# ZheyuanXie/CUDA-Path-Tracer-Denoising

Measured on AMD Instinct MI355X. Metric: SVGF Mpixels/s (full pipeline) at 1080p; à-trous HBM GB/s vs roofline, higher is better.
Workload: dtype f32; 1 GPU; cornell-like 1920x1080, full SVGF (temporal + 5 a-trous levels, history_level 1), static camera, steady-state history; one independent sequence per GPU; width=1920, height=1080, atrous_levels=5, parallelism=replicas1

## Files before the change

### cuda-path-tracer-denoising_amd/csrc/svgf_kernels.h

```cpp
#pragma once
#include <hip/hip_runtime.h>
#include <hip/hip_ext.h>
#include <mutex>

#ifdef SVGF_BUILD_EXPERIMENTS
int svgf_exp_get(const char *name, int dflt);
#define SVGF_TUNE(name, dflt) svgf_exp_get(name, dflt)
#else
#define SVGF_TUNE(name, dflt) (dflt)
#endif

struct SvgfLaunchEvents { hipEvent_t start, stop; };
extern thread_local SvgfLaunchEvents g_svgf_launch_events;
#define SVGF_LAUNCH_KERNEL(kernel, grid, block, lds, stream, ...)                                                        \
    do {                                                                                                                 \
        if (g_svgf_launch_events.start) {                                                                                \
            const SvgfLaunchEvents ev__ = g_svgf_launch_events;                                                          \
            g_svgf_launch_events = SvgfLaunchEvents{ nullptr, nullptr };                                                 \
            hipExtLaunchKernelGGL(kernel, grid, block, lds, stream, ev__.start, ev__.stop, 0, __VA_ARGS__);              \
        } else {                                                                                                         \
            hipLaunchKernelGGL(kernel, grid, block, lds, stream, __VA_ARGS__);                                           \
        }                                                                                                                \
    } while (0)

// ... 35 lines not shown
    float4 *dst;
    float *out_rgb;
    const float *nrm;
    const float *pos;
    const float *gbuf;
    const float *albedo;
    int W, H, step;
    float sigma_c, sigma_n, sigma_x;
    int blur_variance;
    int modulate;
    const float *var;
    float *var_dst;
    const float4 *tin;
    float4 *tout;
    int t_m, t_m_out;
};

struct TemporalArgs {
    const float *in_rgb;
    const float *gbuf;
    const float4 *cv_hist;
    float4 *cv_acc;
    const float2 *mom_hist; float2 *mom_acc;
    const int *hlen; int *hlen_upd;
    const float *nrm_prev; const int *gid_prev;
    float *nrm_cur; int *gid_cur; float *pos_cur;
    float M[16];
    int W, H;
    float color_alpha_min, moment_alpha_min;
    float reproj_sx, reproj_sy;
    const float *pos_prev;
    float pos_tol;
    void *dump;
    const void *arena;
    size_t arena_bytes;
    int skip_split;
    const void *motion;
    int motion_format;
    int clamp_radius;
    float clamp_k;
    const float *xf;
    int n_geoms;
    int firefly_rank;
    float firefly_scale;
};

#define SVGF_MOTION_FMT_NONE  0
#define SVGF_MOTION_FMT_COORD 1
#define SVGF_MOTION_FMT_D32   2
#define SVGF_MOTION_FMT_D16   3
#define SVGF_MOTION_FMT_RUNTIME (-1)
hipError_t launch_temporal(const TemporalArgs &a, hipStream_t s);
bool       temporal_motion_format_known(int motion_format);
bool       temporal_clamp_supported(int W, int H);
struct MotionReprojArgs {
    void *out;
    int format;
    const float *gbuf;
    const float *pos;
    const int *gid;
    float M[16];
    int W, H;
    float reproj_sx, reproj_sy;
    const float *xf;
    int n_geoms;
};
hipError_t launch_motion_reproject(const MotionReprojArgs &a, hipStream_t s);
struct OutputTaaArgs {
    const float *pre;
    float *out;
    const float4 *hist;
    float4 *hist_new;
    const float *pos;
    const int *gid;
    const void *motion;
    int motion_format;
    const float *xf;
    int n_geoms;
    float M[16];
    int W, H;
    float reproj_sx, reproj_sy;
    float alpha, k;
};
hipError_t launch_output_taa(const OutputTaaArgs &a, hipStream_t s);
hipError_t launch_spatial_variance(float4 *cv_acc, const float2 *mom_acc, const int *hlen_upd, const float *nrm, const int *gid,
                                   int W, int H, int K, hipStream_t s);
hipError_t launch_prepare(const float *in_rgb, const float *gbuf, float4 *cv, float *nrm, int *gid, float *pos,
                          int W, int H, hipStream_t s);
hipError_t launch_prepare_filtered(const float *in_rgb, const float *gbuf, float4 *cv, float *nrm, int *gid, float *pos,
                                   int W, int H, int rank, float scale, hipStream_t s);
hipError_t launch_atrous_gather(const AtrousArgs &a, hipStream_t s);
hipError_t launch_atrous_strip(const AtrousArgs &a, hipStream_t s);
hipError_t launch_atrous_lane(const AtrousArgs &a, hipStream_t s);
hipError_t launch_atrous_prepare_fused(const AtrousArgs &a, const TemporalArgs &t, hipStream_t s);
bool       atrous_prepare_fused_supported(const AtrousArgs &a, const TemporalArgs &t);
#ifdef SVGF_BUILD_EXPERIMENTS
hipError_t launch_atrous_lane_reuse(const AtrousArgs &a, hipStream_t s);
hipError_t launch_atrous_fused(const AtrousArgs &a, const TemporalArgs &t, hipStream_t s);
bool       atrous_fused_supported(const AtrousArgs &a, const TemporalArgs &t);
hipError_t launch_atrous_split_fused(const AtrousArgs &a, const TemporalArgs &t, hipStream_t s);
bool       atrous_split_fused_supported(const AtrousArgs &a, const TemporalArgs &t);
hipError_t launch_atrous_lane_2y(const AtrousArgs &a, hipStream_t s);
void atrous_lane_block(const AtrousArgs &a, int *threads, int *lds_bytes);
void atrous_lane2y_block(bool fused, int *threads, int *lds_bytes);
#endif
hipError_t launch_atrous_lattice(const AtrousArgs &a, hipStream_t s);
// ... 15 lines not shown
```

### cuda-path-tracer-denoising_amd/csrc/svgf_kernels.hip

```cpp
#include "svgf_kernels.h"
#include "svgf_temporal.h"

#define SVGF_BLOCK 256

static inline int div_up(long long a, int b) { return (int)((a + b - 1) / b); }


__device__ __forceinline__ float lum_strict(float r, float g, float b) { return svgf_lum_strict(r, g, b); }
__device__ __forceinline__ float dist3_strict(float ax, float ay, float az, float bx, float by, float bz) { return svgf_dist3_strict(ax, ay, az, bx, by, bz); }


__device__ __forceinline__ int reproj_valid(const TemporalArgs &a, float qx, float qy, int gid, float nx, float ny, float nz)
{
    const int q = svgf_tap_index(a, qx, qy);
    if (q < 0) return -1;
    const int gq = a.gid_prev[q];
    if (gq == -1 || gq != gid) return -1;
    const float *n = a.nrm_prev + 3 * (size_t)q;
    return svgf_normals_close(n[0], n[1], n[2], nx, ny, nz) ? q : -1;
}

__device__ __forceinline__ int reproj_valid_pos(const TemporalArgs &a, int q, float px, float py, float pz)
{
    if (q < 0 || !(a.pos_tol > 0.0f)) return q;
    const float *pp = a.pos_prev + 3 * (size_t)q;
    return (dist3_strict(pp[0], pp[1], pp[2], px, py, pz) <= a.pos_tol) ? q : -1;
}

#define SVGF_CLAMP_TILE_W 64
#define SVGF_CLAMP_TILE_H (SVGF_BLOCK / SVGF_CLAMP_TILE_W)
template <int R> struct ClampTile {
    static constexpr int PITCH = SVGF_CLAMP_TILE_W + 2 * R, ROWS = SVGF_CLAMP_TILE_H + 2 * R, PLANE = PITCH * ROWS;
    const float *c0, *c1, *c2;
    int x, y;
};

template <int BLOCK, int MOTION, bool XF>
__global__ __launch_bounds__(BLOCK) void k_temporal(TemporalArgs a)
{
#pragma clang fp contract(off)
    const int n = a.W * a.H;
    const int p = blockIdx.x * BLOCK + threadIdx.x;
    if (p >= n) return;
    constexpr int R = 0;
    constexpr bool FILTERED = false;
    const ClampTile<R> tile = {};
#include "svgf_temporal_pixel.inc.h"
}

template <int BLOCK, int MOTION, bool XF, int R>
__global__ __launch_bounds__(BLOCK) void k_temporal_clamped(TemporalArgs a)
{
#pragma clang fp contract(off)
    typedef ClampTile<R> T;
    static_assert(BLOCK == SVGF_CLAMP_TILE_W * SVGF_CLAMP_TILE_H, "one thread per pixel of the tile");
    __shared__ float lds[3 * T::PLANE];
    const int x0 = blockIdx.x * SVGF_CLAMP_TILE_W, y0 = blockIdx.y * SVGF_CLAMP_TILE_H;
    for (int j = threadIdx.x; j < 3 * T::PLANE; j += BLOCK) {
        const int row = j / (3 * T::PITCH), k = j - row * (3 * T::PITCH), col = k / 3, ch = k - 3 * col;
        const int gx = x0 - R + col, gy = y0 - R + row;
        float v = 0.0f;
        if (gx >= 0 && gx < a.W && gy >= 0 && gy < a.H) v = a.in_rgb[3 * ((size_t)gy * a.W + gx) + ch];
        lds[ch * T::PLANE + row * T::PITCH + col] = v;
    }
    __syncthreads();
    const int tx = threadIdx.x % SVGF_CLAMP_TILE_W, ty = threadIdx.x / SVGF_CLAMP_TILE_W;
    T tile;
    tile.x = x0 + tx; tile.y = y0 + ty;
    if (tile.x >= a.W || tile.y >= a.H) return;
    tile.c0 = lds + (ty + R) * T::PITCH + (tx + R); tile.c1 = tile.c0 + T::PLANE; tile.c2 = tile.c1 + T::PLANE;
    const int p = tile.x + tile.y * a.W;
    constexpr bool FILTERED = false;
#include "svgf_temporal_pixel.inc.h"
}

template <int M> struct FireflyRaw {
    static constexpr int PITCH = SVGF_CLAMP_TILE_W + 2 * M, ROWS = SVGF_CLAMP_TILE_H + 2 * M, PLANE = PITCH * ROWS;
};
template <int BLOCK, int M>
__device__ __forceinline__ void firefly_stage(float *raw, const float *__restrict__ in_rgb, int x0, int y0, int W, int H)
{
    typedef FireflyRaw<M> S;
    for (int j = threadIdx.x; j < S::PLANE; j += BLOCK) {
        const int row = j / S::PITCH, col = j - row * S::PITCH;
        const int gx = x0 - M + col, gy = y0 - M + row;
        float r = 0.0f, g = 0.0f, b = 0.0f;
        if (gx >= 0 && gx < W && gy >= 0 && gy < H) {
            const float *c = in_rgb + 3 * ((size_t)gy * W + gx);
            r = c[0]; g = c[1]; b = c[2];
        }
        raw[j] = r; raw[S::PLANE + j] = g; raw[2 * S::PLANE + j] = b;
        raw[3 * S::PLANE + j] = lum_strict(r, g, b);
    }
}

template <int BLOCK, int R>
__global__ __launch_bounds__(BLOCK) void k_temporal_filtered(TemporalArgs a)
{
#pragma clang fp contract(off)
    typedef ClampTile<R> T;
    typedef FireflyRaw<R + 1> S;
    static_assert(BLOCK == SVGF_CLAMP_TILE_W * SVGF_CLAMP_TILE_H, "one thread per pixel of the tile");
    __shared__ float raw[4 * S::PLANE];
    __shared__ float lds[3 * T::PLANE];
    const int x0 = blockIdx.x * SVGF_CLAMP_TILE_W, y0 = blockIdx.y * SVGF_CLAMP_TILE_H;
    firefly_stage<BLOCK, R + 1>(raw, a.in_rgb, x0, y0, a.W, a.H);
    __syncthreads();
    for (int j = threadIdx.x; j < T::PLANE; j += BLOCK) {
        const int row = j / T::PITCH, col = j - row * T::PITCH;
        const int gx = x0 - R + col, gy = y0 - R + row;
        float r = 0.0f, g = 0.0f, b = 0.0f;
        if (gx >= 0 && gx < a.W && gy >= 0 && gy < a.H) {
            const int o = (row + 1) * S::PITCH + (col + 1);
            r = raw[o]; g = raw[S::PLANE + o]; b = raw[2 * S::PLANE + o];
            svgf_firefly_filter<S::PITCH>(raw + 3 * S::PLANE + o, gx, gy, a.W, a.H, a.firefly_rank, a.firefly_scale, r, g, b);
        }
        lds[j] = r; lds[T::PLANE + j] = g; lds[2 * T::PLANE + j] = b;
    }
    __syncthreads();
    const int tx = threadIdx.x % SVGF_CLAMP_TILE_W, ty = threadIdx.x / SVGF_CLAMP_TILE_W;
    T tile;
    tile.x = x0 + tx; tile.y = y0 + ty;
    if (tile.x >= a.W || tile.y >= a.H) return;
    tile.c0 = lds + (ty + R) * T::PITCH + (tx + R); tile.c1 = tile.c0 + T::PLANE; tile.c2 = tile.c1 + T::PLANE;
    const int p = tile.x + tile.y * a.W;
    constexpr bool FILTERED = true, XF = true;
    constexpr int MOTION = SVGF_MOTION_FMT_RUNTIME;
#include "svgf_temporal_pixel.inc.h"
}

static hipError_t launch_temporal_filtered(const TemporalArgs &a, hipStream_t s)
{
    if (a.firefly_rank < 1 || a.firefly_rank > 3 || !temporal_clamp_supported(a.W, a.H)) return hipErrorInvalidValue;
    if (a.motion && !temporal_motion_format_known(a.motion_format)) return hipErrorInvalidValue;
    const dim3 grid(div_up(a.W, SVGF_CLAMP_TILE_W), div_up(a.H, SVGF_CLAMP_TILE_H)), block(SVGF_BLOCK);
    switch (a.clamp_radius) {
    case 0: SVGF_LAUNCH_KERNEL((k_temporal_filtered<SVGF_BLOCK, 0>), grid, block, 0, s, a); break;
    case 1: SVGF_LAUNCH_KERNEL((k_temporal_filtered<SVGF_BLOCK, 1>), grid, block, 0, s, a); break;
    case 2: SVGF_LAUNCH_KERNEL((k_temporal_filtered<SVGF_BLOCK, 2>), grid, block, 0, s, a); break;
    case 3: SVGF_LAUNCH_KERNEL((k_temporal_filtered<SVGF_BLOCK, 3>), grid, block, 0, s, a); break;
    default: return hipErrorInvalidValue;
    }
    return hipGetLastError();
}

template <int MOTION, bool XF>
static hipError_t launch_temporal_clamped(const TemporalArgs &a, hipStream_t s)
{
    const dim3 grid(div_up(a.W, SVGF_CLAMP_TILE_W), div_up(a.H, SVGF_CLAMP_TILE_H)), block(SVGF_BLOCK);
    switch (a.clamp_radius) {
    case 1: SVGF_LAUNCH_KERNEL((k_temporal_clamped<SVGF_BLOCK, MOTION, XF, 1>), grid, block, 0, s, a); break;
    case 2: SVGF_LAUNCH_KERNEL((k_temporal_clamped<SVGF_BLOCK, MOTION, XF, 2>), grid, block, 0, s, a); break;
    case 3: SVGF_LAUNCH_KERNEL((k_temporal_clamped<SVGF_BLOCK, MOTION, XF, 3>), grid, block, 0, s, a); break;
    default: return hipErrorInvalidValue;
    }
    return hipGetLastError();
}

bool temporal_clamp_supported(int W, int H) { (void)W; return H <= 65535 * SVGF_CLAMP_TILE_H; }

template <bool XF>
static hipError_t launch_temporal_xf(const TemporalArgs &a, hipStream_t s)
{
    if (a.clamp_radius != 0) {
        if (!temporal_clamp_supported(a.W, a.H)) return hipErrorInvalidValue;
        if (!a.motion) return launch_temporal_clamped<SVGF_MOTION_FMT_NONE, XF>(a, s);
        switch (a.motion_format) {
        case SVGF_MOTION_FMT_COORD: return launch_temporal_clamped<SVGF_MOTION_FMT_COORD, XF>(a, s);
        case SVGF_MOTION_FMT_D32:   return launch_temporal_clamped<SVGF_MOTION_FMT_D32, XF>(a, s);
        case SVGF_MOTION_FMT_D16:   return launch_temporal_clamped<SVGF_MOTION_FMT_D16, XF>(a, s);
        default: return hipErrorInvalidValue;
        }
    }
    const long long n = (long long)a.W * a.H;
    const dim3 grid(div_up(n, SVGF_BLOCK)), block(SVGF_BLOCK);
    if (!a.motion) {
        SVGF_LAUNCH_KERNEL((k_temporal<SVGF_BLOCK, SVGF_MOTION_FMT_NONE, XF>), grid, block, 0, s, a);
        return hipGetLastError();
    }
    switch (a.motion_format) {
    case SVGF_MOTION_FMT_COORD: SVGF_LAUNCH_KERNEL((k_temporal<SVGF_BLOCK, SVGF_MOTION_FMT_COORD, XF>), grid, block, 0, s, a); break;
    case SVGF_MOTION_FMT_D32:   SVGF_LAUNCH_KERNEL((k_temporal<SVGF_BLOCK, SVGF_MOTION_FMT_D32, XF>), grid, block, 0, s, a); break;
    case SVGF_MOTION_FMT_D16:   SVGF_LAUNCH_KERNEL((k_temporal<SVGF_BLOCK, SVGF_MOTION_FMT_D16, XF>), grid, block, 0, s, a); break;
    default: return hipErrorInvalidValue;
    }
    return hipGetLastError();
}

hipError_t launch_temporal(const TemporalArgs &a, hipStream_t s)
{
    if (a.firefly_rank != 0) return launch_temporal_filtered(a, s);
    return (a.xf && a.n_geoms > 0) ? launch_temporal_xf<true>(a, s) : launch_temporal_xf<false>(a, s);
}

bool temporal_motion_format_known(int f) { return f == SVGF_MOTION_FMT_COORD || f == SVGF_MOTION_FMT_D32 || f == SVGF_MOTION_FMT_D16; }

__global__ __launch_bounds__(SVGF_BLOCK) void k_motion_reproject(MotionReprojArgs a)
{
#pragma clang fp contract(off)
    const int n = a.W * a.H;
    const int p = blockIdx.x * SVGF_BLOCK + threadIdx.x;
    if (p >= n) return;
    float px, py, pz;
    int gid;
    if (a.gbuf) {
        const float *t = a.gbuf + 13 * (size_t)p;
        px = t[3]; py = t[4]; pz = t[5];
        gid = __float_as_int(t[12]);
    } else {
        px = a.pos[3 * (size_t)p]; py = a.pos[3 * (size_t)p + 1]; pz = a.pos[3 * (size_t)p + 2];
        gid = a.gid[p];
    }
    float ox, oy;
    if (gid == -1) {
        ox = oy = __uint_as_float(0x7fc00000u);
    } else {
        if (a.xf && gid >= 0 && gid < a.n_geoms) {
            const float *m = a.xf + 12 * (size_t)gid;
            float q[3];
#pragma unroll
            for (int r = 0; r < 3; r++) {
                float t0 = m[4 * r] * px + m[4 * r + 1] * py;
                t0 = t0 + m[4 * r + 2] * pz;
                q[r] = t0 + m[4 * r + 3];
            }
            px = q[0]; py = q[1]; pz = q[2];
        }
        const SvgfPrevCoord c = svgf_project_prev(a.M, a.W, a.H, a.reproj_sx, a.reproj_sy, px, py, pz);
        ox = c.x; oy = c.y;
        if (a.format != SVGF_MOTION_FMT_COORD) {
            const int y = p / a.W, x = p - y * a.W;
            ox = ox - (float)x; oy = oy - (float)y;
        }
    }
    if (a.format == SVGF_MOTION_FMT_D16) ((__half2 *)a.out)[p] = __halves2half2(__float2half(ox), __float2half(oy));
    else ((float2 *)a.out)[p] = make_float2(ox, oy);
}

hipError_t launch_motion_reproject(const MotionReprojArgs &a, hipStream_t s)
{
    const long long n = (long long)a.W * a.H;
    SVGF_LAUNCH_KERNEL(k_motion_reproject, dim3(div_up(n, SVGF_BLOCK)), dim3(SVGF_BLOCK), 0, s, a);
    return hipGetLastError();
}
// ... 297 lines not shown
```

### cuda-path-tracer-denoising_amd/csrc/svgf_temporal.h

```cpp
#pragma once
#include <hip/hip_fp16.h>
#include "svgf_kernels.h"

__device__ __forceinline__ float svgf_lum_strict(float r, float g, float b)
{
#pragma clang fp contract(off)
    double l = 0.2126 * (double)r + 0.7152 * (double)g;
    l = l + 0.0722 * (double)b;
    return (float)l;
}

__device__ __forceinline__ float svgf_dist3_strict(float ax, float ay, float az, float bx, float by, float bz)
{
#pragma clang fp contract(off)
    float dx = bx - ax, dy = by - ay, dz = bz - az;
    float s = dx * dx + dy * dy;
    s = s + dz * dz;
    return sqrtf(s);
}

struct SvgfPrevCoord { float x, y; };
__device__ __forceinline__ SvgfPrevCoord svgf_project_prev(const float *M, int W, int H, float reproj_sx, float reproj_sy,
                                                           float px, float py, float pz)
{
#pragma clang fp contract(off)
    float vs[3];
#pragma unroll
    for (int r = 0; r < 3; r++) {
        float a0 = M[0 * 4 + r] * px + M[1 * 4 + r] * py;
        float a1 = M[2 * 4 + r] * pz + M[3 * 4 + r] * 1.0f;
        vs[r] = a0 + a1;
    }
    float clipx = vs[0] / vs[2], clipy = vs[1] / vs[2];
    if (reproj_sx > 0.0f) clipx = clipx / reproj_sx;
    if (reproj_sy > 0.0f) clipy = clipy / reproj_sy;
    float ndcx = -clipx * 0.5f + 0.5f, ndcy = -clipy * 0.5f + 0.5f;
    SvgfPrevCoord c;
    c.x = ndcx * (float)W - 0.5f; c.y = ndcy * (float)H - 0.5f;
    return c;
}

struct SvgfReproj { float fx, fy, fracx, fracy; };
__device__ __forceinline__ SvgfReproj svgf_reproj_from_coord(float prevx, float prevy)
{
#pragma clang fp contract(off)
    SvgfReproj r;
    r.fx = floorf(prevx); r.fy = floorf(prevy);
    r.fracx = prevx - r.fx; r.fracy = prevy - r.fy;
    return r;
}
__device__ __forceinline__ bool svgf_reproj_on_screen(const TemporalArgs &a, const SvgfReproj &r)
{
    return r.fx >= 0.0f && r.fy >= 0.0f && r.fx < (float)a.W && r.fy < (float)a.H;
}

__device__ __forceinline__ SvgfReproj svgf_reproject(const TemporalArgs &a, float px, float py, float pz)
{
    const SvgfPrevCoord c = svgf_project_prev(a.M, a.W, a.H, a.reproj_sx, a.reproj_sy, px, py, pz);
    return svgf_reproj_from_coord(c.x, c.y);
}

template <int FORMAT>
__device__ __forceinline__ SvgfPrevCoord svgf_motion_prev_coord(const TemporalArgs &a, int p)
{
#pragma clang fp contract(off)
    SvgfPrevCoord c;
    if constexpr (FORMAT == SVGF_MOTION_FMT_COORD) {
        const float2 m = ((const float2 *)a.motion)[p];
        c.x = m.x; c.y = m.y;
    } else {
        const int y = p / a.W, x = p - y * a.W;
        float dx, dy;
        if constexpr (FORMAT == SVGF_MOTION_FMT_D32) {
            const float2 m = ((const float2 *)a.motion)[p];
            dx = m.x; dy = m.y;
        } else {
            const __half2 m = ((const __half2 *)a.motion)[p];
            dx = __low2float(m); dy = __high2float(m);
        }
        c.x = (float)x + dx; c.y = (float)y + dy;
    }
    return c;
}

__device__ __forceinline__ void svgf_to_prev_space(const float *xf, int gid, float &px, float &py, float &pz, float &nx, float &ny, float &nz)
{
#pragma clang fp contract(off)
    const float4 *m = (const float4 *)xf + 3 * (size_t)gid;
    float q[3], n[3];
#pragma unroll
    for (int r = 0; r < 3; r++) {
        const float4 row = m[r];
        float t0 = row.x * px + row.y * py;
        t0 = t0 + row.z * pz;
        q[r] = t0 + row.w;
        float t1 = row.x * nx + row.y * ny;
        n[r] = t1 + row.z * nz;
    }
    px = q[0]; py = q[1]; pz = q[2];
    nx = n[0]; ny = n[1]; nz = n[2];
}

__device__ __forceinline__ int svgf_tap_index(const TemporalArgs &a, float qx, float qy)
{
    if (!(qx == qx) || !(qy == qy)) return -1;
    if (qx < 0.0f || qx >= (float)a.W || qy < 0.0f || qy >= (float)a.H) return -1;
    return (int)qx + (int)qy * a.W;
}

__device__ __forceinline__ bool svgf_normals_close(float nqx, float nqy, float nqz, float nx, float ny, float nz)
{
#pragma clang fp contract(off)
    const float dx = nx - nqx, dy = ny - nqy, dz = nz - nqz;
    float s = dx * dx + dy * dy;
    s = s + dz * dz;
    return !(s > __uint_as_float(0x3c23d70bu));
}
__device__ __forceinline__ bool svgf_tap_consistent(int gq, float nqx, float nqy, float nqz, int gid, float nx, float ny, float nz)
{
    return (gq != -1) & (gq == gid) & svgf_normals_close(nqx, nqy, nqz, nx, ny, nz);
}

__device__ __forceinline__ void svgf_bilinear_weights(float fracx, float fracy, float (&w)[4])
{
#pragma clang fp contract(off)
    w[0] = (1 - fracx) * (1 - fracy); w[1] = fracx * (1 - fracy); w[2] = (1 - fracx) * fracy; w[3] = fracx * fracy;
}

struct SvgfHistSum { float pc0, pc1, pc2, pm0, pm1, plen; };
__device__ __forceinline__ void svgf_hist_add_weighted(SvgfHistSum &h, float w, float c0, float c1, float c2, float m0, float m1, int len)
{
#pragma clang fp contract(off)
    h.pc0 += w * c0; h.pc1 += w * c1; h.pc2 += w * c2;
    h.pm0 += w * m0; h.pm1 += w * m1;
    h.plen += w * (float)len;
}
__device__ __forceinline__ void svgf_hist_add(SvgfHistSum &h, float c0, float c1, float c2, float m0, float m1, int len)
{
#pragma clang fp contract(off)
    h.pc0 += c0; h.pc1 += c1; h.pc2 += c2;
    h.pm0 += m0; h.pm1 += m1;
    h.plen += (float)len;
}
__device__ __forceinline__ void svgf_hist_div(SvgfHistSum &h, float d)
{
#pragma clang fp contract(off)
    h.pc0 /= d; h.pc1 /= d; h.pc2 /= d; h.pm0 /= d; h.pm1 /= d; h.plen /= d;
}

__device__ __forceinline__ float svgf_clamp_to_box(float pc, float m, float q, float n, float k)
{
#pragma clang fp contract(off)
    const float sd = sqrtf(q / n);
    const float ksd = k * sd;
    const float lo = m - ksd, hi = m + ksd;
    if (pc < lo) pc = lo;
    if (pc > hi) pc = hi;
    return pc;
}
template <int R, int PITCH>
__device__ __forceinline__ void svgf_history_clamp(SvgfHistSum &h, const float *c0, const float *c1, const float *c2,
                                                   int x, int y, int W, int H, float k)
{
#pragma clang fp contract(off)
    bool in_y[2 * R + 1], in_x[2 * R + 1];
#pragma unroll
    for (int d = -R; d <= R; d++) {
        in_y[d + R] = (unsigned)(y + d) < (unsigned)H;
        in_x[d + R] = (unsigned)(x + d) < (unsigned)W;
    }
    float n = 0.0f, s0 = 0.0f, s1 = 0.0f, s2 = 0.0f;
#pragma unroll
    for (int yy = -R; yy <= R; yy++)
#pragma unroll
        for (int xx = -R; xx <= R; xx++)
            if (in_y[yy + R] && in_x[xx + R]) {
                const int o = yy * PITCH + xx;
                s0 += c0[o]; s1 += c1[o]; s2 += c2[o];
                n += 1.0f;
            }
    const float m0 = s0 / n, m1 = s1 / n, m2 = s2 / n;
    float q0 = 0.0f, q1 = 0.0f, q2 = 0.0f;
#pragma unroll
    for (int yy = -R; yy <= R; yy++)
#pragma unroll
        for (int xx = -R; xx <= R; xx++)
            if (in_y[yy + R] && in_x[xx + R]) {
                const int o = yy * PITCH + xx;
                const float d0 = c0[o] - m0, d1 = c1[o] - m1, d2 = c2[o] - m2;
                q0 += d0 * d0; q1 += d1 * d1; q2 += d2 * d2;
            }
    h.pc0 = svgf_clamp_to_box(h.pc0, m0, q0, n, k);
    h.pc1 = svgf_clamp_to_box(h.pc1, m1, q1, n, k);
    h.pc2 = svgf_clamp_to_box(h.pc2, m2, q2, n, k);
}

template <int PITCH>
__device__ __forceinline__ void svgf_firefly_filter(const float *lum, int x, int y, int W, int H, int rank, float scale,
                                                    float &r, float &g, float &b)
{
#pragma clang fp contract(off)
    const float ninf = __uint_as_float(0xff800000u);
    float t0 = ninf, t1 = ninf, t2 = ninf;
    int n = 0;
#pragma unroll
    for (int yy = -1; yy <= 1; yy++)
#pragma unroll
        for (int xx = -1; xx <= 1; xx++) {
            if (xx == 0 && yy == 0) continue;
            if ((unsigned)(x + xx) < (unsigned)W && (unsigned)(y + yy) < (unsigned)H) {
                float v = lum[yy * PITCH + xx];
                if (v == v) {
                    n += 1;
                    if (v > t0) { const float u = t0; t0 = v; v = u; }
                    if (rank > 1 && v > t1) { const float u = t1; t1 = v; v = u; }
                    if (rank > 2 && v > t2) { const float u = t2; t2 = v; v = u; }
                }
            }
        }
    if (n == 0) return;
    const int k = rank < n ? rank : n;
    const float B = k <= 1 ? t0 : (k == 2 ? t1 : t2);
    const float bound = scale * B;
    const float Lp = lum[0];
    if (Lp > bound) {
        const float s = bound / Lp;
        r = r * s; g = g * s; b = b * s;
    }
}

struct SvgfTemporalOut { float4 cv; float2 mom; int hlen; };
__device__ __forceinline__ SvgfTemporalOut svgf_temporal_blend(const TemporalArgs &a, float cr, float cg, float cb, float lum, int N,
                                                              bool valid, const SvgfHistSum &hs)
{
#pragma clang fp contract(off)
    const float pc0 = hs.pc0, pc1 = hs.pc1, pc2 = hs.pc2, pm0 = hs.pm0, pm1 = hs.pm1, plen = hs.plen;
    SvgfTemporalOut o;
    if (valid) {
        const float ca = fmaxf(1.0f / (float)(N + 1), a.color_alpha_min);
        const float ma = fmaxf(1.0f / (float)(N + 1), a.moment_alpha_min);
        o.hlen = (int)plen + 1;
        const float m1 = ma * pm0 + (1.0f - ma) * lum;
        const float m2 = ma * pm1 + ((1.0f - ma) * lum) * lum;
        o.mom = make_float2(m1, m2);
        const float v = m2 - m1 * m1;
        o.cv = make_float4(cr * ca + pc0 * (1.0f - ca), cg * ca + pc1 * (1.0f - ca), cb * ca + pc2 * (1.0f - ca), v > 0.0f ? v : 0.0f);
    } else {
        o.hlen = 1;
        o.mom = make_float2(lum, lum * lum);
        o.cv = make_float4(cr, cg, cb, 100.0f);
    }
    return o;
}
```

### cuda-path-tracer-denoising_amd/csrc/svgf_temporal_pixel.inc.h

```cpp
    float nx, ny, nz, px, py, pz;
    int gid;
    if (a.gbuf) {
        const float *t = a.gbuf + 13 * (size_t)p;
        nx = t[0]; ny = t[1]; nz = t[2];
        px = t[3]; py = t[4]; pz = t[5];
        gid = __float_as_int(t[12]);
        if (!a.skip_split) {
            a.nrm_cur[3 * (size_t)p] = nx; a.nrm_cur[3 * (size_t)p + 1] = ny; a.nrm_cur[3 * (size_t)p + 2] = nz;
            a.pos_cur[3 * (size_t)p] = px; a.pos_cur[3 * (size_t)p + 1] = py; a.pos_cur[3 * (size_t)p + 2] = pz;
            a.gid_cur[p] = gid;
        }
    } else {
        nx = a.nrm_cur[3 * (size_t)p]; ny = a.nrm_cur[3 * (size_t)p + 1]; nz = a.nrm_cur[3 * (size_t)p + 2];
        px = a.pos_cur[3 * (size_t)p]; py = a.pos_cur[3 * (size_t)p + 1]; pz = a.pos_cur[3 * (size_t)p + 2];
        gid = a.gid_cur[p];
    }

    float cr, cg, cb;
    if constexpr (R > 0 || FILTERED) {
        cr = *tile.c0; cg = *tile.c1; cb = *tile.c2;
    } else {
        cr = a.in_rgb[3 * (size_t)p]; cg = a.in_rgb[3 * (size_t)p + 1]; cb = a.in_rgb[3 * (size_t)p + 2];
    }
    const float lum = lum_strict(cr, cg, cb);
    const int N = a.hlen[p];

    bool valid = false;
    SvgfHistSum hs = { 0.0f, 0.0f, 0.0f, 0.0f, 0.0f, 0.0f };
    if (N > 0 && gid != -1) {
        float tnx = nx, tny = ny, tnz = nz, tpx = px, tpy = py, tpz = pz;
        if constexpr (XF) {
            if (gid >= 0 && gid < a.n_geoms) svgf_to_prev_space(a.xf, gid, tpx, tpy, tpz, tnx, tny, tnz);
        }
        SvgfReproj rp;
        if constexpr (MOTION == SVGF_MOTION_FMT_NONE) {
            rp = svgf_reproject(a, tpx, tpy, tpz);
        } else if constexpr (MOTION == SVGF_MOTION_FMT_RUNTIME) {
            if (!a.motion) {
                rp = svgf_reproject(a, tpx, tpy, tpz);
            } else {
                SvgfPrevCoord c;
                switch (a.motion_format) {
                case SVGF_MOTION_FMT_COORD: c = svgf_motion_prev_coord<SVGF_MOTION_FMT_COORD>(a, p); break;
                case SVGF_MOTION_FMT_D32:   c = svgf_motion_prev_coord<SVGF_MOTION_FMT_D32>(a, p); break;
                default:                    c = svgf_motion_prev_coord<SVGF_MOTION_FMT_D16>(a, p); break;
                }
                rp = svgf_reproj_from_coord(c.x, c.y);
            }
        } else {
            const SvgfPrevCoord c = svgf_motion_prev_coord<MOTION>(a, p);
            rp = svgf_reproj_from_coord(c.x, c.y);
        }
        const float fx = rp.fx, fy = rp.fy;

        valid = svgf_reproj_on_screen(a, rp);
        int q4[4];
#pragma unroll
        for (int k = 0; k < 4; k++) {
            q4[k] = reproj_valid_pos(a, reproj_valid(a, fx + (float)(k & 1), fy + (float)(k >> 1), gid, tnx, tny, tnz), tpx, tpy, tpz);
            valid = valid && (q4[k] >= 0);
        }

        if (valid) {
            float w[4];
            svgf_bilinear_weights(rp.fracx, rp.fracy, w);
            float sumw = 0.0f;
#pragma unroll
            for (int k = 0; k < 4; k++) {
                const int q = q4[k];
                const float4 ch = a.cv_hist[q];
                const float2 mh = a.mom_hist[q];
                svgf_hist_add_weighted(hs, w[k], ch.x, ch.y, ch.z, mh.x, mh.y, a.hlen[q]);
                sumw += w[k];
            }
            if ((double)sumw >= 0.01) svgf_hist_div(hs, sumw);
        } else {
            float cnt = 0.0f;
            for (int yy = -1; yy <= 1; yy++)
                for (int xx = -1; xx <= 1; xx++) {
                    const int q = (xx >= 0 && yy >= 0) ? q4[xx + 2 * yy]
                                                       : reproj_valid_pos(a, reproj_valid(a, fx + (float)xx, fy + (float)yy, gid, tnx, tny, tnz), tpx, tpy, tpz);
                    if (q >= 0) {
                        const float4 ch = a.cv_hist[q];
                        const float2 mh = a.mom_hist[q];
                        svgf_hist_add(hs, ch.x, ch.y, ch.z, mh.x, mh.y, a.hlen[q]);
                        cnt += 1.0f;
                    }
                }
            if (cnt > 0.0f) {
                svgf_hist_div(hs, cnt);
                valid = true;
            }
        }
        if constexpr (R > 0) {
            if (valid) svgf_history_clamp<R, ClampTile<R>::PITCH>(hs, tile.c0, tile.c1, tile.c2, tile.x, tile.y, a.W, a.H, a.clamp_k);
        }
    }
    const SvgfTemporalOut o = svgf_temporal_blend(a, cr, cg, cb, lum, N, valid, hs);
    a.hlen_upd[p] = o.hlen;
    a.mom_acc[p] = o.mom;
    a.cv_acc[p] = o.cv;
```

Baseline: 9073 Mpixels/s.

## Optimize temporal reprojection with 32-bit offsets, batched tap loads, shared-reciprocal division

The temporal kernel now uses 32-bit byte offsets whenever the frame is small enough, and a separate wide-offset fallback variant handles large frames. The four bilinear reprojection taps are validated with batched, branch-free loads (gid, then normal, then position) instead of per-tap dependent calls. Per-pixel IEEE divisions (projection divide, history normalisation, 1/(N+1)) are replaced by a shared-reciprocal Newton sequence when every lane in the wavefront is in a safe range. The aim is to cut address arithmetic, load latency chains and divide cost in the temporal pass. The price is extra code complexity and a reliance on bit-exactness arguments for the custom division.

```diff
diff --git a/cuda-path-tracer-denoising_amd/csrc/svgf_kernels.h b/cuda-path-tracer-denoising_amd/csrc/svgf_kernels.h
--- a/cuda-path-tracer-denoising_amd/csrc/svgf_kernels.h
+++ b/cuda-path-tracer-denoising_amd/csrc/svgf_kernels.h
@@ -111,6 +111,7 @@
 #define SVGF_MOTION_FMT_RUNTIME (-1)
 hipError_t launch_temporal(const TemporalArgs &a, hipStream_t s);
 bool       temporal_motion_format_known(int motion_format);
+bool       temporal_wide_offsets(int W, int H, bool aos);
 bool       temporal_clamp_supported(int W, int H);
 struct MotionReprojArgs {
     void *out;
diff --git a/cuda-path-tracer-denoising_amd/csrc/svgf_kernels.hip b/cuda-path-tracer-denoising_amd/csrc/svgf_kernels.hip
--- a/cuda-path-tracer-denoising_amd/csrc/svgf_kernels.hip
+++ b/cuda-path-tracer-denoising_amd/csrc/svgf_kernels.hip
@@ -10,20 +10,24 @@
 __device__ __forceinline__ float dist3_strict(float ax, float ay, float az, float bx, float by, float bz) { return svgf_dist3_strict(ax, ay, az, bx, by, bz); }
 
 
+template <bool WIDE>
 __device__ __forceinline__ int reproj_valid(const TemporalArgs &a, float qx, float qy, int gid, float nx, float ny, float nz)
 {
+    typedef typename SvgfOffset<WIDE>::type toff;
     const int q = svgf_tap_index(a, qx, qy);
     if (q < 0) return -1;
-    const int gq = a.gid_prev[q];
+    const int gq = *svgf_at(a.gid_prev, (toff)q * 4u);
     if (gq == -1 || gq != gid) return -1;
-    const float *n = a.nrm_prev + 3 * (size_t)q;
+    const float *n = svgf_at(a.nrm_prev, (toff)q * 12u);
     return svgf_normals_close(n[0], n[1], n[2], nx, ny, nz) ? q : -1;
 }
 
+template <bool WIDE>
 __device__ __forceinline__ int reproj_valid_pos(const TemporalArgs &a, int q, float px, float py, float pz)
 {
+    typedef typename SvgfOffset<WIDE>::type toff;
     if (q < 0 || !(a.pos_tol > 0.0f)) return q;
-    const float *pp = a.pos_prev + 3 * (size_t)q;
+    const float *pp = svgf_at(a.pos_prev, (toff)q * 12u);
     return (dist3_strict(pp[0], pp[1], pp[2], px, py, pz) <= a.pos_tol) ? q : -1;
 }
 
@@ -35,7 +39,7 @@
     int x, y;
 };
 
-template <int BLOCK, int MOTION, bool XF>
+template <int BLOCK, int MOTION, bool XF, bool WIDE>
 __global__ __launch_bounds__(BLOCK) void k_temporal(TemporalArgs a)
 {
 #pragma clang fp contract(off)
@@ -48,7 +52,7 @@
 #include "svgf_temporal_pixel.inc.h"
 }
 
-template <int BLOCK, int MOTION, bool XF, int R>
+template <int BLOCK, int MOTION, bool XF, int R, bool WIDE>
 __global__ __launch_bounds__(BLOCK) void k_temporal_clamped(TemporalArgs a)
 {
 #pragma clang fp contract(off)
@@ -94,7 +98,7 @@
     }
 }
 
-template <int BLOCK, int R>
+template <int BLOCK, int R, bool WIDE>
 __global__ __launch_bounds__(BLOCK) void k_temporal_filtered(TemporalArgs a)
 {
 #pragma clang fp contract(off)
@@ -129,29 +133,31 @@
 #include "svgf_temporal_pixel.inc.h"
 }
 
+template <bool WIDE>
 static hipError_t launch_temporal_filtered(const TemporalArgs &a, hipStream_t s)
 {
     if (a.firefly_rank < 1 || a.firefly_rank > 3 || !temporal_clamp_supported(a.W, a.H)) return hipErrorInvalidValue;
     if (a.motion && !temporal_motion_format_known(a.motion_format)) return hipErrorInvalidValue;
     const dim3 grid(div_up(a.W, SVGF_CLAMP_TILE_W), div_up(a.H, SVGF_CLAMP_TILE_H)), block(SVGF_BLOCK);
     switch (a.clamp_radius) {
-    case 0: SVGF_LAUNCH_KERNEL((k_temporal_filtered<SVGF_BLOCK, 0>), grid, block, 0, s, a); break;
-    case 1: SVGF_LAUNCH_KERNEL((k_temporal_filtered<SVGF_BLOCK, 1>), grid, block, 0, s, a); break;
-    case 2: SVGF_LAUNCH_KERNEL((k_temporal_filtered<SVGF_BLOCK, 2>), grid, block, 0, s, a); break;
-    case 3: SVGF_LAUNCH_KERNEL((k_temporal_filtered<SVGF_BLOCK, 3>), grid, block, 0, s, a); break;
+    case 0: SVGF_LAUNCH_KERNEL((k_temporal_filtered<SVGF_BLOCK, 0, WIDE>), grid, block, 0, s, a); break;
+    case 1: SVGF_LAUNCH_KERNEL((k_temporal_filtered<SVGF_BLOCK, 1, WIDE>), grid, block, 0, s, a); break;
+    case 2: SVGF_LAUNCH_KERNEL((k_temporal_filtered<SVGF_BLOCK, 2, WIDE>), grid, block, 0, s, a); break;
+    case 3: SVGF_LAUNCH_KERNEL((k_temporal_filtered<SVGF_BLOCK, 3, WIDE>), grid, block, 0, s, a); break;
     default: return hipErrorInvalidValue;
     }
     return hipGetLastError();
 }
 
-template <int MOTION, bool XF>
+template <int MOTION, bool XF, bool WIDE>
 static hipError_t launch_temporal_clamped(const TemporalArgs &a, hipStream_t s)
 {
+    if (!temporal_clamp_supported(a.W, a.H)) return hipErrorInvalidValue;
     const dim3 grid(div_up(a.W, SVGF_CLAMP_TILE_W), div_up(a.H, SVGF_CLAMP_TILE_H)), block(SVGF_BLOCK);
     switch (a.clamp_radius) {
-    case 1: SVGF_LAUNCH_KERNEL((k_temporal_clamped<SVGF_BLOCK, MOTION, XF, 1>), grid, block, 0, s, a); break;
-    case 2: SVGF_LAUNCH_KERNEL((k_temporal_clamped<SVGF_BLOCK, MOTION, XF, 2>), grid, block, 0, s, a); break;
-    case 3: SVGF_LAUNCH_KERNEL((k_temporal_clamped<SVGF_BLOCK, MOTION, XF, 3>), grid, block, 0, s, a); break;
+    case 1: SVGF_LAUNCH_KERNEL((k_temporal_clamped<SVGF_BLOCK, MOTION, XF, 1, WIDE>), grid, block, 0, s, a); break;
+    case 2: SVGF_LAUNCH_KERNEL((k_temporal_clamped<SVGF_BLOCK, MOTION, XF, 2, WIDE>), grid, block, 0, s, a); break;
+    case 3: SVGF_LAUNCH_KERNEL((k_temporal_clamped<SVGF_BLOCK, MOTION, XF, 3, WIDE>), grid, block, 0, s, a); break;
     default: return hipErrorInvalidValue;
     }
     return hipGetLastError();
@@ -163,33 +169,52 @@
 static hipError_t launch_temporal_xf(const TemporalArgs &a, hipStream_t s)
 {
     if (a.clamp_radius != 0) {
-        if (!temporal_clamp_supported(a.W, a.H)) return hipErrorInvalidValue;
-        if (!a.motion) return launch_temporal_clamped<SVGF_MOTION_FMT_NONE, XF>(a, s);
+        if (!a.motion) return launch_temporal_clamped<SVGF_MOTION_FMT_NONE, XF, false>(a, s);
         switch (a.motion_format) {
-        case SVGF_MOTION_FMT_COORD: return launch_temporal_clamped<SVGF_MOTION_FMT_COORD, XF>(a, s);
-        case SVGF_MOTION_FMT_D32:   return launch_temporal_clamped<SVGF_MOTION_FMT_D32, XF>(a, s);
-        case SVGF_MOTION_FMT_D16:   return launch_temporal_clamped<SVGF_MOTION_FMT_D16, XF>(a, s);
+        case SVGF_MOTION_FMT_COORD: return launch_temporal_clamped<SVGF_MOTION_FMT_COORD, XF, false>(a, s);
+        case SVGF_MOTION_FMT_D32:   return launch_temporal_clamped<SVGF_MOTION_FMT_D32, XF, false>(a, s);
+        case SVGF_MOTION_FMT_D16:   return launch_temporal_clamped<SVGF_MOTION_FMT_D16, XF, false>(a, s);
         default: return hipErrorInvalidValue;
         }
     }
     const long long n = (long long)a.W * a.H;
     const dim3 grid(div_up(n, SVGF_BLOCK)), block(SVGF_BLOCK);
     if (!a.motion) {
-        SVGF_LAUNCH_KERNEL((k_temporal<SVGF_BLOCK, SVGF_MOTION_FMT_NONE, XF>), grid, block, 0, s, a);
+        SVGF_LAUNCH_KERNEL((k_temporal<SVGF_BLOCK, SVGF_MOTION_FMT_NONE, XF, false>), grid, block, 0, s, a);
         return hipGetLastError();
     }
     switch (a.motion_format) {
-    case SVGF_MOTION_FMT_COORD: SVGF_LAUNCH_KERNEL((k_temporal<SVGF_BLOCK, SVGF_MOTION_FMT_COORD, XF>), grid, block, 0, s, a); break;
-    case SVGF_MOTION_FMT_D32:   SVGF_LAUNCH_KERNEL((k_temporal<SVGF_BLOCK, SVGF_MOTION_FMT_D32, XF>), grid, block, 0, s, a); break;
-    case SVGF_MOTION_FMT_D16:   SVGF_LAUNCH_KERNEL((k_temporal<SVGF_BLOCK, SVGF_MOTION_FMT_D16, XF>), grid, block, 0, s, a); break;
+    case SVGF_MOTION_FMT_COORD: SVGF_LAUNCH_KERNEL((k_temporal<SVGF_BLOCK, SVGF_MOTION_FMT_COORD, XF, false>), grid, block, 0, s, a); break;
+    case SVGF_MOTION_FMT_D32:   SVGF_LAUNCH_KERNEL((k_temporal<SVGF_BLOCK, SVGF_MOTION_FMT_D32, XF, false>), grid, block, 0, s, a); break;
+    case SVGF_MOTION_FMT_D16:   SVGF_LAUNCH_KERNEL((k_temporal<SVGF_BLOCK, SVGF_MOTION_FMT_D16, XF, false>), grid, block, 0, s, a); break;
     default: return hipErrorInvalidValue;
     }
     return hipGetLastError();
 }
 
+static hipError_t launch_temporal_wide(TemporalArgs a, hipStream_t s)
+{
+    if (a.motion && !temporal_motion_format_known(a.motion_format)) return hipErrorInvalidValue;
+    if (!a.xf || a.n_geoms < 0) a.n_geoms = 0;
+    if (a.firefly_rank != 0) return launch_temporal_filtered<true>(a, s);
+    if (a.clamp_radius != 0) return launch_temporal_clamped<SVGF_MOTION_FMT_RUNTIME, true, true>(a, s);
+    const long long n = (long long)a.W * a.H;
+    SVGF_LAUNCH_KERNEL((k_temporal<SVGF_BLOCK, SVGF_MOTION_FMT_RUNTIME, true, true>), dim3(div_up(n, SVGF_BLOCK)), dim3(SVGF_BLOCK), 0, s, a);
+    return hipGetLastError();
+}
+
+bool temporal_wide_offsets(int W, int H, bool aos)
+{
+    return (unsigned long long)(aos ? 52 : 16) * (unsigned long long)W * (unsigned long long)H > 0xffffffffull;
+}
+#ifdef SVGF_BUILD_EXPERIMENTS
+extern "C" int svgf_exp_temporal_wide_offsets(int W, int H, int aos) { return temporal_wide_offsets(W, H, aos != 0) ? 1 : 0; }
+#endif
+
 hipError_t launch_temporal(const TemporalArgs &a, hipStream_t s)
 {
-    if (a.firefly_rank != 0) return launch_temporal_filtered(a, s);
+    if (temporal_wide_offsets(a.W, a.H, a.gbuf != nullptr) || SVGF_TUNE("temporal_wide_offsets", 0)) return launch_temporal_wide(a, s);
+    if (a.firefly_rank != 0) return launch_temporal_filtered<false>(a, s);
     return (a.xf && a.n_geoms > 0) ? launch_temporal_xf<true>(a, s) : launch_temporal_xf<false>(a, s);
 }
 
diff --git a/cuda-path-tracer-denoising_amd/csrc/svgf_temporal.h b/cuda-path-tracer-denoising_amd/csrc/svgf_temporal.h
--- a/cuda-path-tracer-denoising_amd/csrc/svgf_temporal.h
+++ b/cuda-path-tracer-denoising_amd/csrc/svgf_temporal.h
@@ -1,6 +1,15 @@
 #pragma once
 #include <hip/hip_fp16.h>
+#include <type_traits>
 #include "svgf_kernels.h"
+
+template <bool WIDE> struct SvgfOffset { typedef typename std::conditional<WIDE, size_t, unsigned>::type type; };
+template <typename T, typename O> __device__ __forceinline__ T *svgf_at(T *base, O byte_off)
+{
+    typedef typename std::conditional<std::is_const<T>::value, const char, char>::type B;
+    if constexpr (sizeof(O) == 4) asm("" : "+v"(byte_off));
+    return reinterpret_cast<T *>(reinterpret_cast<B *>(base) + byte_off);
+}
 
 __device__ __forceinline__ float svgf_lum_strict(float r, float g, float b)
 {
@@ -19,6 +28,31 @@
     return sqrtf(s);
 }
 
+#define SVGF_DIV_LO_BITS 0x2b800000u
+#define SVGF_DIV_LO __uint_as_float(SVGF_DIV_LO_BITS)
+#define SVGF_DIV_HI __uint_as_float(0x53800000u)
+__device__ __forceinline__ bool svgf_every_lane(bool ok) { return __builtin_amdgcn_ballot_w64(!ok) == 0; }
+struct SvgfDivisor { float d, r1; };
+__device__ __forceinline__ SvgfDivisor svgf_div_shared_prepare(float d)
+{
+    const float r = __builtin_amdgcn_rcpf(d);
+    const float e0 = __builtin_fmaf(-d, r, 1.0f);
+    return SvgfDivisor{ d, __builtin_fmaf(e0, r, r) };
+}
+__device__ __forceinline__ float svgf_div_shared_nofix(const SvgfDivisor &c, float a)
+{
+#pragma clang fp contract(off)
+    const float q0 = a * c.r1;
+    const float e1 = __builtin_fmaf(-c.d, q0, a);
+    const float q1 = __builtin_fmaf(e1, c.r1, q0);
+    const float e2 = __builtin_fmaf(-c.d, q1, a);
+    return __builtin_fmaf(e2, c.r1, q1);
+}
+__device__ __forceinline__ float svgf_div_shared(const SvgfDivisor &c, float a)
+{
+    return __builtin_amdgcn_div_fixupf(svgf_div_shared_nofix(c, a), c.d, a);
+}
+
 struct SvgfPrevCoord { float x, y; };
 __device__ __forceinline__ SvgfPrevCoord svgf_project_prev(const float *M, int W, int H, float reproj_sx, float reproj_sy,
                                                            float px, float py, float pz)
@@ -31,9 +65,19 @@
         float a1 = M[2 * 4 + r] * pz + M[3 * 4 + r] * 1.0f;
         vs[r] = a0 + a1;
     }
-    float clipx = vs[0] / vs[2], clipy = vs[1] / vs[2];
-    if (reproj_sx > 0.0f) clipx = clipx / reproj_sx;
-    if (reproj_sy > 0.0f) clipy = clipy / reproj_sy;
+    float clipx, clipy;
+    {
+        const float a0 = fabsf(vs[0]), a1 = fabsf(vs[1]), a2 = fabsf(vs[2]);
+        const bool ok = fminf(fminf(a0, a1), a2) >= SVGF_DIV_LO && fmaxf(fmaxf(a0, a1), a2) <= SVGF_DIV_HI;
+        if (svgf_every_lane(ok)) {
+            const SvgfDivisor c = svgf_div_shared_prepare(vs[2]);
+            clipx = svgf_div_shared_nofix(c, vs[0]); clipy = svgf_div_shared_nofix(c, vs[1]);
+        } else {
+            clipx = vs[0] / vs[2]; clipy = vs[1] / vs[2];
+        }
+    }
+    if (reproj_sx > 0.0f) { asm volatile(""); clipx = clipx / reproj_sx; }
+    if (reproj_sy > 0.0f) { asm volatile(""); clipy = clipy / reproj_sy; }
     float ndcx = -clipx * 0.5f + 0.5f, ndcy = -clipy * 0.5f + 0.5f;
     SvgfPrevCoord c;
     c.x = ndcx * (float)W - 0.5f; c.y = ndcy * (float)H - 0.5f;
@@ -60,22 +104,22 @@
     return svgf_reproj_from_coord(c.x, c.y);
 }
 
-template <int FORMAT>
+template <int FORMAT, typename O = size_t>
 __device__ __forceinline__ SvgfPrevCoord svgf_motion_prev_coord(const TemporalArgs &a, int p)
 {
 #pragma clang fp contract(off)
     SvgfPrevCoord c;
     if constexpr (FORMAT == SVGF_MOTION_FMT_COORD) {
-        const float2 m = ((const float2 *)a.motion)[p];
+        const float2 m = *svgf_at((const float2 *)a.motion, (O)p * 8u);
         c.x = m.x; c.y = m.y;
     } else {
         const int y = p / a.W, x = p - y * a.W;
         float dx, dy;
         if constexpr (FORMAT == SVGF_MOTION_FMT_D32) {
-            const float2 m = ((const float2 *)a.motion)[p];
+            const float2 m = *svgf_at((const float2 *)a.motion, (O)p * 8u);
             dx = m.x; dy = m.y;
         } else {
-            const __half2 m = ((const __half2 *)a.motion)[p];
+            const __half2 m = *svgf_at((const __half2 *)a.motion, (O)p * 4u);
             dx = __low2float(m); dy = __high2float(m);
         }
         c.x = (float)x + dx; c.y = (float)y + dy;
@@ -108,13 +152,18 @@
     return (int)qx + (int)qy * a.W;
 }
 
-__device__ __forceinline__ bool svgf_normals_close(float nqx, float nqy, float nqz, float nx, float ny, float nz)
+__device__ __forceinline__ float svgf_normal_dist2(float nqx, float nqy, float nqz, float nx, float ny, float nz)
 {
 #pragma clang fp contract(off)
     const float dx = nx - nqx, dy = ny - nqy, dz = nz - nqz;
     float s = dx * dx + dy * dy;
     s = s + dz * dz;
-    return !(s > __uint_as_float(0x3c23d70bu));
+    return s;
+}
+__device__ __forceinline__ bool svgf_dist2_close(float s) { return !(s > __uint_as_float(0x3c23d70bu)); }
+__device__ __forceinline__ bool svgf_normals_close(float nqx, float nqy, float nqz, float nx, float ny, float nz)
+{
+    return svgf_dist2_close(svgf_normal_dist2(nqx, nqy, nqz, nx, ny, nz));
 }
 __device__ __forceinline__ bool svgf_tap_consistent(int gq, float nqx, float nqy, float nqz, int gid, float nx, float ny, float nz)
 {
@@ -147,6 +196,25 @@
 #pragma clang fp contract(off)
     h.pc0 /= d; h.pc1 /= d; h.pc2 /= d; h.pm0 /= d; h.pm1 /= d; h.plen /= d;
 }
+
+__device__ __forceinline__ void svgf_hist_div_shared(SvgfHistSum &h, float d)
+{
+#pragma clang fp contract(off)
+    auto key = [](float v) { return (__float_as_uint(v) << 1) - 1u; };
+    const float top = fmaxf(fmaxf(fmaxf(fabsf(h.pc0), fabsf(h.pc1)), fabsf(h.pc2)), fmaxf(fmaxf(fabsf(h.pm0), fabsf(h.pm1)), fabsf(h.plen)));
+    const unsigned bot = min(min(min(key(h.pc0), key(h.pc1)), key(h.pc2)), min(min(key(h.pm0), key(h.pm1)), key(h.plen)));
+    const float ad = fabsf(d);
+    const bool ok = ad >= SVGF_DIV_LO && ad <= SVGF_DIV_HI && !(top > SVGF_DIV_HI) && bot >= (SVGF_DIV_LO_BITS << 1) - 1u;
+    if (svgf_every_lane(ok)) {
+        const SvgfDivisor c = svgf_div_shared_prepare(d);
+        h.pc0 = svgf_div_shared(c, h.pc0); h.pc1 = svgf_div_shared(c, h.pc1); h.pc2 = svgf_div_shared(c, h.pc2);
+        h.pm0 = svgf_div_shared(c, h.pm0); h.pm1 = svgf_div_shared(c, h.pm1); h.plen = svgf_div_shared(c, h.plen);
+    } else {
+        svgf_hist_div(h, d);
+    }
+}
+
+__device__ __forceinline__ bool svgf_weights_usable(float sumw) { return sumw >= __uint_as_float(0x3c23d70bu); }
 
 __device__ __forceinline__ float svgf_clamp_to_box(float pc, float m, float q, float n, float k)
 {
@@ -234,11 +302,12 @@
                                                               bool valid, const SvgfHistSum &hs)
 {
 #pragma clang fp contract(off)
-    const float pc0 = hs.pc0, pc1 = hs.pc1, pc2 = hs.pc2, pm0 = hs.pm0, pm1 = hs.pm1, plen = hs.plen;
     SvgfTemporalOut o;
     if (valid) {
-        const float ca = fmaxf(1.0f / (float)(N + 1), a.color_alpha_min);
-        const float ma = fmaxf(1.0f / (float)(N + 1), a.moment_alpha_min);
+        const float pc0 = hs.pc0, pc1 = hs.pc1, pc2 = hs.pc2, pm0 = hs.pm0, pm1 = hs.pm1, plen = hs.plen;
+        const float inv = (N >= 1) ? svgf_div_shared_nofix(svgf_div_shared_prepare((float)(N + 1)), 1.0f) : 1.0f / (float)(N + 1);
+        const float ca = fmaxf(inv, a.color_alpha_min);
+        const float ma = fmaxf(inv, a.moment_alpha_min);
         o.hlen = (int)plen + 1;
         const float m1 = ma * pm0 + (1.0f - ma) * lum;
         const float m2 = ma * pm1 + ((1.0f - ma) * lum) * lum;
diff --git a/cuda-path-tracer-denoising_amd/csrc/svgf_temporal_pixel.inc.h b/cuda-path-tracer-denoising_amd/csrc/svgf_temporal_pixel.inc.h
--- a/cuda-path-tracer-denoising_amd/csrc/svgf_temporal_pixel.inc.h
+++ b/cuda-path-tracer-denoising_amd/csrc/svgf_temporal_pixel.inc.h
@@ -1,32 +1,36 @@
+    typedef typename SvgfOffset<WIDE>::type toff;
+    const toff b4 = (toff)p * 4u, b12 = (toff)p * 12u;
     float nx, ny, nz, px, py, pz;
     int gid;
     if (a.gbuf) {
-        const float *t = a.gbuf + 13 * (size_t)p;
+        const float *t = svgf_at(a.gbuf, (toff)p * 52u);
         nx = t[0]; ny = t[1]; nz = t[2];
         px = t[3]; py = t[4]; pz = t[5];
         gid = __float_as_int(t[12]);
         if (!a.skip_split) {
-            a.nrm_cur[3 * (size_t)p] = nx; a.nrm_cur[3 * (size_t)p + 1] = ny; a.nrm_cur[3 * (size_t)p + 2] = nz;
-            a.pos_cur[3 * (size_t)p] = px; a.pos_cur[3 * (size_t)p + 1] = py; a.pos_cur[3 * (size_t)p + 2] = pz;
-            a.gid_cur[p] = gid;
+            float *n = svgf_at(a.nrm_cur, b12), *q = svgf_at(a.pos_cur, b12);
+            n[0] = nx; n[1] = ny; n[2] = nz;
+            q[0] = px; q[1] = py; q[2] = pz;
+            *svgf_at(a.gid_cur, b4) = gid;
         }
     } else {
-        nx = a.nrm_cur[3 * (size_t)p]; ny = a.nrm_cur[3 * (size_t)p + 1]; nz = a.nrm_cur[3 * (size_t)p + 2];
-        px = a.pos_cur[3 * (size_t)p]; py = a.pos_cur[3 * (size_t)p + 1]; pz = a.pos_cur[3 * (size_t)p + 2];
-        gid = a.gid_cur[p];
+        const float *n = svgf_at(a.nrm_cur, b12), *q = svgf_at(a.pos_cur, b12);
+        nx = n[0]; ny = n[1]; nz = n[2];
+        px = q[0]; py = q[1]; pz = q[2];
+        gid = *svgf_at(a.gid_cur, b4);
     }
 
     float cr, cg, cb;
     if constexpr (R > 0 || FILTERED) {
         cr = *tile.c0; cg = *tile.c1; cb = *tile.c2;
     } else {
-        cr = a.in_rgb[3 * (size_t)p]; cg = a.in_rgb[3 * (size_t)p + 1]; cb = a.in_rgb[3 * (size_t)p + 2];
+        const float *c = svgf_at(a.in_rgb, b12);
+        cr = c[0]; cg = c[1]; cb = c[2];
     }
-    const float lum = lum_strict(cr, cg, cb);
-    const int N = a.hlen[p];
+    const int N = *svgf_at(a.hlen, b4);
 
     bool valid = false;
-    SvgfHistSum hs = { 0.0f, 0.0f, 0.0f, 0.0f, 0.0f, 0.0f };
+    SvgfHistSum hs;
     if (N > 0 && gid != -1) {
         float tnx = nx, tny = ny, tnz = nz, tpx = px, tpy = py, tpz = pz;
         if constexpr (XF) {
@@ -41,62 +45,106 @@
             } else {
                 SvgfPrevCoord c;
                 switch (a.motion_format) {
-                case SVGF_MOTION_FMT_COORD: c = svgf_motion_prev_coord<SVGF_MOTION_FMT_COORD>(a, p); break;
-                case SVGF_MOTION_FMT_D32:   c = svgf_motion_prev_coord<SVGF_MOTION_FMT_D32>(a, p); break;
-                default:                    c = svgf_motion_prev_coord<SVGF_MOTION_FMT_D16>(a, p); break;
+                case SVGF_MOTION_FMT_COORD: c = svgf_motion_prev_coord<SVGF_MOTION_FMT_COORD, toff>(a, p); break;
+                case SVGF_MOTION_FMT_D32:   c = svgf_motion_prev_coord<SVGF_MOTION_FMT_D32, toff>(a, p); break;
+                default:                    c = svgf_motion_prev_coord<SVGF_MOTION_FMT_D16, toff>(a, p); break;
                 }
                 rp = svgf_reproj_from_coord(c.x, c.y);
             }
         } else {
-            const SvgfPrevCoord c = svgf_motion_prev_coord<MOTION>(a, p);
+            const SvgfPrevCoord c = svgf_motion_prev_coord<MOTION, toff>(a, p);
             rp = svgf_reproj_from_coord(c.x, c.y);
         }
         const float fx = rp.fx, fy = rp.fy;
 
-        valid = svgf_reproj_on_screen(a, rp);
-        int q4[4];
+        const float Wf = (float)a.W, Hf = (float)a.H;
+        const float fx1 = fx + 1.0f, fy1 = fy + 1.0f;
+        const bool in_x[2] = { fx >= 0.0f && fx < Wf, fx1 >= 0.0f && fx1 < Wf };
+        const bool in_y[2] = { fy >= 0.0f && fy < Hf, fy1 >= 0.0f && fy1 < Hf };
+        const int q00 = (int)fminf(fmaxf(fx, -1.0f), Wf) + (int)fminf(fmaxf(fy, -1.0f), Hf) * a.W;
+        const int qa[4] = { q00, q00 + 1, q00 + a.W, q00 + a.W + 1 };
+        bool ok[4];
+        {
+            int gq[4];
 #pragma unroll
-        for (int k = 0; k < 4; k++) {
-            q4[k] = reproj_valid_pos(a, reproj_valid(a, fx + (float)(k & 1), fy + (float)(k >> 1), gid, tnx, tny, tnz), tpx, tpy, tpz);
-            valid = valid && (q4[k] >= 0);
+            for (int k = 0; k < 4; k++) {
+                ok[k] = in_x[k & 1] && in_y[k >> 1];
+                gq[k] = *svgf_at(a.gid_prev, ok[k] ? (toff)qa[k] * 4u : (toff)0);
+            }
+            float nq[4][3];
+#pragma unroll
+            for (int k = 0; k < 4; k++) {
+                ok[k] = ok[k] && gq[k] == gid;
+                const float *n = svgf_at(a.nrm_prev, ok[k] ? (toff)qa[k] * 12u : (toff)0);
+                nq[k][0] = n[0]; nq[k][1] = n[1]; nq[k][2] = n[2];
+            }
+#pragma unroll
+            for (int k = 0; k < 4; k++) {
+                const float s = svgf_normal_dist2(nq[k][0], nq[k][1], nq[k][2], tnx, tny, tnz);
+                ok[k] = ok[k] && svgf_dist2_close(s);
+            }
         }
+        int q00b = q00;
+        asm("" : "+v"(q00b));
+        const int q4[4] = { q00b, q00b + 1, q00b + a.W, q00b + a.W + 1 };
+        if (a.pos_tol > 0.0f) {
+            float pq[4][3];
+#pragma unroll
+            for (int k = 0; k < 4; k++) {
+                const float *pp = svgf_at(a.pos_prev, ok[k] ? (toff)q4[k] * 12u : (toff)0);
+                pq[k][0] = pp[0]; pq[k][1] = pp[1]; pq[k][2] = pp[2];
+            }
+#pragma unroll
+            for (int k = 0; k < 4; k++) {
+                const float d = dist3_strict(pq[k][0], pq[k][1], pq[k][2], tpx, tpy, tpz);
+                ok[k] = ok[k] && d <= a.pos_tol;
+            }
+        }
+        valid = ok[0] && ok[1] && ok[2] && ok[3];
 
+        float divisor;
+        bool divide;
         if (valid) {
+            hs = SvgfHistSum{ 0.0f, 0.0f, 0.0f, 0.0f, 0.0f, 0.0f };
             float w[4];
             svgf_bilinear_weights(rp.fracx, rp.fracy, w);
             float sumw = 0.0f;
 #pragma unroll
             for (int k = 0; k < 4; k++) {
-                const int q = q4[k];
-                const float4 ch = a.cv_hist[q];
-                const float2 mh = a.mom_hist[q];
-                svgf_hist_add_weighted(hs, w[k], ch.x, ch.y, ch.z, mh.x, mh.y, a.hlen[q]);
+                const toff q = (toff)q4[k & 2];
+                const float4 ch = svgf_at(a.cv_hist, q * 16u)[k & 1];
+                const float2 mh = svgf_at(a.mom_hist, q * 8u)[k & 1];
+                svgf_hist_add_weighted(hs, w[k], ch.x, ch.y, ch.z, mh.x, mh.y, svgf_at(a.hlen, q * 4u)[k & 1]);
                 sumw += w[k];
             }
-            if ((double)sumw >= 0.01) svgf_hist_div(hs, sumw);
+            divisor = sumw;
+            divide = svgf_weights_usable(sumw);
         } else {
+            hs = SvgfHistSum{ 0.0f, 0.0f, 0.0f, 0.0f, 0.0f, 0.0f };
             float cnt = 0.0f;
             for (int yy = -1; yy <= 1; yy++)
                 for (int xx = -1; xx <= 1; xx++) {
-                    const int q = (xx >= 0 && yy >= 0) ? q4[xx + 2 * yy]
-                                                       : reproj_valid_pos(a, reproj_valid(a, fx + (float)xx, fy + (float)yy, gid, tnx, tny, tnz), tpx, tpy, tpz);
-                    if (q >= 0) {
-                        const float4 ch = a.cv_hist[q];
-                        const float2 mh = a.mom_hist[q];
-                        svgf_hist_add(hs, ch.x, ch.y, ch.z, mh.x, mh.y, a.hlen[q]);
+                    int qi;
+                    if (xx >= 0 && yy >= 0) qi = ok[xx + 2 * yy] ? q4[xx + 2 * yy] : -1;
+                    else qi = reproj_valid_pos<WIDE>(a, reproj_valid<WIDE>(a, fx + (float)xx, fy + (float)yy, gid, tnx, tny, tnz), tpx, tpy, tpz);
+                    if (qi >= 0) {
+                        const toff q = (toff)qi;
+                        const float4 ch = *svgf_at(a.cv_hist, q * 16u);
+                        const float2 mh = *svgf_at(a.mom_hist, q * 8u);
+                        svgf_hist_add(hs, ch.x, ch.y, ch.z, mh.x, mh.y, *svgf_at(a.hlen, q * 4u));
                         cnt += 1.0f;
                     }
                 }
-            if (cnt > 0.0f) {
-                svgf_hist_div(hs, cnt);
-                valid = true;
-            }
+            divisor = cnt;
+            divide = valid = cnt > 0.0f;
         }
+        if (divide) svgf_hist_div_shared(hs, divisor);
         if constexpr (R > 0) {
             if (valid) svgf_history_clamp<R, ClampTile<R>::PITCH>(hs, tile.c0, tile.c1, tile.c2, tile.x, tile.y, a.W, a.H, a.clamp_k);
         }
     }
+    const float lum = lum_strict(cr, cg, cb);
     const SvgfTemporalOut o = svgf_temporal_blend(a, cr, cg, cb, lum, N, valid, hs);
-    a.hlen_upd[p] = o.hlen;
-    a.mom_acc[p] = o.mom;
-    a.cv_acc[p] = o.cv;
+    *svgf_at(a.hlen_upd, b4) = o.hlen;
+    *svgf_at(a.mom_acc, (toff)p * 8u) = o.mom;
+    *svgf_at(a.cv_acc, (toff)p * 16u) = o.cv;
```

Result: no change. 9153 Mpixels/s, median of 6 (+0.9%).
